# ultravideo/kvazaar

Hardware: AMD Instinct MI355X
Metric: CTUs/s (all-intra ultrafast hot path) (higher is better)
Workload: dtype u8/i16 (f64 RD costs); 1 GPU; 1920x1080 yuv420p 8-bit all-intra ultrafast CTU pass (kvz_hip_intra_frames), QP 22; ctus_per_frame=510, distinct_frames=8, wpp=True, parallelism=frames sharded over 1 GPU(s), no data-path collective

## Files before the change

### include/kvz_hip_dev.h

```cpp
#ifndef KVZ_HIP_DEV_H_
#define KVZ_HIP_DEV_H_

#include "kvz_hip_types.h"

#ifdef __cplusplus
extern "C" {
#endif

void *kvz_hip_dev_alloc(size_t bytes);
void  kvz_hip_dev_free(void *p);
void  kvz_hip_dev_upload(void *dev_dst, const void *host_src, size_t bytes);
void  kvz_hip_dev_download(void *host_dst, const void *dev_src, size_t bytes);
void  kvz_hip_dev_sync(void);
void  kvz_hip_dev_copy(void *dev_dst, const void *dev_src, size_t bytes);
void  kvz_hip_dev_timer_start(void);
float kvz_hip_dev_timer_stop(void);

int  kvz_hip_dev_sad_nxn(int n, const uint8_t *a, const uint8_t *b, int count, uint32_t *out);
int  kvz_hip_dev_satd_nxn(int n, const uint8_t *a, const uint8_t *b, int count, uint32_t *out);

int  kvz_hip_dev_transform(int kind, const int16_t *in, int16_t *tmp, int16_t *out, int count, int use_matrix_cores);

int  kvz_hip_dev_angular_pred(int log2_width, int mode, const uint8_t *ref_above, const uint8_t *ref_left, int count, uint8_t *out);

int  kvz_hip_dev_intra_select(int log2w, int nblk, const uint32_t *raw, const int8_t *preds, const double *mode_bits, int count, int32_t *winner);

int  kvz_hip_dev_cu8_units(int count, int from_coeffs, const int16_t *in, const int32_t *qp, int16_t *levels, int16_t *dequant, int16_t *resid);

int  kvz_hip_dev_satd8_blocks(const uint8_t *a, const uint8_t *b, int count, uint32_t *out);

void kvz_hip_dev_deblock_frames(uint8_t *frames, int width, int height, int n_frames, const uint8_t *cu_depth, int qp, int beta_offset_div2,
                                int tc_offset_div2);

typedef struct kvz_hip_cu_dbk {
  uint8_t type;
  uint8_t depth, tr_depth, part_size;
  uint8_t cbf_y;
  uint8_t mv_dir;
  int8_t  mv_ref[2];
  int16_t ref_id[2];
  int16_t mv[2][2];
} kvz_hip_cu_dbk;
void kvz_hip_dev_deblock_frames_inter(uint8_t *frames, int width, int height, int n_frames, const kvz_hip_cu_dbk *info, int qp, int beta_offset_div2,
                                      int tc_offset_div2, int slice_is_b);
// ... 131 lines not shown
```

### kvazaar_amd/csrc/kvz_ctu.hpp

```cpp
#pragma once
#include <type_traits>
#include "../../include/kvz_hip_types.h"
#include "kvz_ops.hpp"
#include "kvz_rdoq.hpp"
#include "kvz_recon.hpp"
#include "kvz_residual.hpp"
#include "kvz_select.hpp"

namespace kvz {

#define KVZ_CTU_THREADS 128
#ifdef KVZ_HOSTSIM
#define KVZ_FOR_THREADS(tid) for (int tid = 0; tid < KVZ_CTU_THREADS; ++tid)
#ifdef KVZ_HOSTSIM_COUNT_SYNCS
static unsigned long long g_kvz_syncs;
#define KVZ_SYNC() (++g_kvz_syncs)
#else
#define KVZ_SYNC()
#endif
#define KVZ_LDS_ADD(p, v) (*(p) += (v))
#else
#define KVZ_FOR_THREADS(tid) for (int tid = (threadIdx.x + lane_rot) & (KVZ_CTU_THREADS - 1), once_ = 1; once_; once_ = 0)
#define KVZ_SYNC() __syncthreads()
#define KVZ_LDS_ADD(p, v) atomicAdd((p), (v))
// ... 180 lines not shown
  u8 *cu_part = nullptr;
  u8 *cu_mode4 = nullptr;
  double *ctu_cost;
  unsigned long long *prof;
  u8 *border;
};
#define KVZ_BORDER_BYTES 512

template <bool CABAC> struct CtuSharedT {
  alignas(16) u8 org[1536];
  alignas(16) u8 dec[6144];
#if defined(KVZ_CTU_PROFILE) && !defined(KVZ_HOSTSIM)
  unsigned long long prof_rq[16];
  unsigned long long prof_acc[96];
  int prof_pu;
#endif
  CtuCu cu[4][64];
  u8 ref[3][2][68];
  u8 fref[2][68];
  union {
    struct {
      alignas(16) i16 tb_big[1536];
      alignas(16) u8 c1[1536];
    };
    struct {
      alignas(16) i16 tb_small[2 * 384];
      alignas(8) u8 org_t[256];
      alignas(16) u8 c2[384];
      alignas(16) i16 lv3_coeff[384];
      u8 mref[15][KVZ_MREF_STRIDE];
      u32 satd_raw[35][4];
    };
  };
  alignas(16) i16 lv2_coeff[384];
  alignas(16) i16 lv1_coeff[1536];
#ifdef KVZ_HOSTSIM
  alignas(16) i16 dct32[32 * 32];
#else
  alignas(16) i16 dct_small[64 + 16];
#endif
  u32 acc[16];
  int8_t preds[3];
  int best_mode;
  double cost[4], split_cost[4];
  double res[4];
  double child_bits[4];
// ... 5 lines not shown
  u8 dcval[3];
  int8_t mode_disp[35];
  int16_t mode_inv[35];
  QuantScalars qs[4][2];
  double mode_bits_cost[3];
  CtxSetT<CABAC> cab, pre[3], post2;
  float entropy_fbits[128];
  u8 ctx_lps[64];
};

using CtuShared = CtuSharedT<true>;
static_assert(__builtin_offsetof(CtuSharedT<true>, fref) == __builtin_offsetof(CtuSharedT<true>, ref) + 408 && __builtin_offsetof(CtuSharedT<false>, fref) == __builtin_offsetof(CtuSharedT<false>, ref) + 408,
              "Tables::mref_tab addresses the filtered references 408 bytes behind the unfiltered ones");
static_assert(KVZ_MREF_STRIDE == kMrefStride && KVZ_MREF_ORG == kMrefOrg && sizeof(((CtuSharedT<true> *)0)->ref[0][0]) == kMrefRefRow && kMrefFiltered == 408,
              "Tables::mref_tab (kvz_tables.hpp) is built for this layout of the reference arrays");
static_assert(KVZ_CTU_THREADS == 128, "two wavefronts per CTU: thread 64 is 'the other wavefront' (recon_cu8, eval_pu, wide_task, rdoq_unit, prices_coeffs, kHookThread), a 16x16 CU's "
                                      "128 (mode, block) pairs are one round of rough_search, plane_sums routes DPP rows per wavefront, and mref_pre[4] covers Tables::mref_tab's 510 entries");

KVZ_HD int plane_off(int c) { return c ? 3072 + (c << 10) : 0; }

struct RdoqLds {
  i32 ptab[2 * 148];
  u8 diag8[64];
  u8 mode4[4][64][4];
  u8 nb_mode4_left[16];
  u8 c4[96];
  alignas(8) i16 lv4_coeff[96];
  u8 pu_mode[4], pu_cbf[4];
  int pu_cbf_c[2];
  int a3x, a3y, n_pu;
// ... 565 lines not shown
        const int c = g < ny ? 0 : 1, i = g - (c == 0 ? 0 : ny);
        const int l2 = c ? log2w_c : log2w_y, n = 2 * (1 << l2) + 1, side = i >= n, k = side ? i - n : i;
        int qx, qy, dv;
        const bool have = ref_coords(l2, c, x, y, side, k, avail_top, avail_left, &qx, &qy);
        const lds_off off = rec_off(lv, c, qx, qy, &dv);
        s->ref[c][side][k] = have ? base[off] : (u8)128;
        if (c) s->ref[2][side][k] = have ? base[off + dv] : (u8)128;
      }
    }
    KVZ_SYNC();
    KVZ_FOR_THREADS(tid) {
      if (luma) {
        const int n = 2 * (1 << log2w_y) + 1;
        for (int i = tid; i < 2 * n; i += KVZ_CTU_THREADS) {
          const int side = i >= n, k = side ? i - n : i;
          const u8 *r = s->ref[0][side];
          u8 v;
          if (k == 0) v = (u8)((s->ref[0][1][1] + 2 * s->ref[0][1][0] + s->ref[0][0][1] + 2) / 4);
          else if (k == n - 1) v = r[k];
          else v = (u8)((r[k - 1] + 2 * r[k] + r[k + 1] + 2) / 4);
          s->fref[side][k] = v;
        }
      }
      const int c = mover_lane(tid) - (KVZ_CTU_THREADS - 3);
      if (c >= 0 && ((c == 0 && luma) || (c > 0 && chroma))) {
        const int l2 = c ? log2w_c : log2w_y, w = 1 << l2;
#ifdef KVZ_HOSTSIM
        s->dcval[c] = (u8)dc_value(l2, s->ref[c][0], s->ref[c][1]);
#else
        u32 sum = 0;
        for (int i = 0; i < w; i += 4) {
          u32 a, b;
          __builtin_memcpy(&a, &s->ref[c][0][1 + i], 4);
          __builtin_memcpy(&b, &s->ref[c][1][1 + i], 4);
          sum = __builtin_amdgcn_sad_u8(a, 0u, sum);
          sum = __builtin_amdgcn_sad_u8(b, 0u, sum);
// ... 44 lines not shown
      int d[8];
      for (int x = 0; x < 8; x++) d[x] = (int)pa[x] - (int)pb[x];
      int u0, u1, u2, u3;
      if (col & 4) { u0 = d[0] - d[4]; u1 = d[1] - d[5]; u2 = d[2] - d[6]; u3 = d[3] - d[7]; }
      else { u0 = d[0] + d[4]; u1 = d[1] + d[5]; u2 = d[2] + d[6]; u3 = d[3] + d[7]; }
      const int v0 = (col & 2) ? u0 - u2 : u0 + u2, v1 = (col & 2) ? u1 - u3 : u1 + u3;
      t[r] = (col & 1) ? v0 - v1 : v0 + v1;
    }
    KVZ_HAD8(t[0], t[1], t[2], t[3], t[4], t[5], t[6], t[7]);
    u32 sum = 0;
    for (int r = 0; r < 8; r++) sum += (u32)iabs(t[r]);
    return sum;
  }

#ifndef KVZ_HOSTSIM
  typedef unsigned short U16x2 __attribute__((ext_vector_type(2)));
  KVZ_DEV static U16x2 u16x2_of(unsigned v) { U16x2 r; __builtin_memcpy(&r, &v, 4); return r; }
  KVZ_DEV static U16x2 splat16(int v) { U16x2 r; r.x = (unsigned short)v; r.y = (unsigned short)v; return r; }
  KVZ_DEV static U16x2 widen(unsigned hi, unsigned lo, unsigned sel) { return u16x2_of(__builtin_amdgcn_perm(hi, lo, sel)); }
  KVZ_DEV static Pk16 as_pk16(U16x2 v) { Pk16 r; __builtin_memcpy(&r, &v, 4); return r; }
  KVZ_DEV static void widen8(const u8 *p, U16x2 out[4])
  {
    unsigned w[2];
    __builtin_memcpy(w, p, 8);
    out[0] = widen(0, w[0], 0x0c010c00u); out[1] = widen(0, w[0], 0x0c030c02u); out[2] = widen(0, w[1], 0x0c010c00u); out[3] = widen(0, w[1], 0x0c030c02u);
  }
#endif
  template <bool PAIR>
  KVZ_DEV u32 angular_block_satd(int log2w, int mode, int bx, int by, int xl, int yl, int half) const
  {
    const int w = 1 << log2w;
    const bool big = S32 && log2w == 5;
    const bool flat = mode < 2;
    const bool vertical = mode >= 18 || flat;
// ... 82 lines not shown
        sum += pk_absmax(pk_add(b0, b1)) + pk_absmax(pk_sub(b0, b1)) + pk_absmax(pk_add(b2, b3)) + pk_absmax(pk_sub(b2, b3));
        sum += pk_absmax(pk_add(b4, b5)) + pk_absmax(pk_sub(b4, b5)) + pk_absmax(pk_add(b6, b7)) + pk_absmax(pk_sub(b6, b7));
#else
        sum = pk_abs2_biased(pk_add(b0, b1), sum); sum = pk_abs2_biased(pk_sub(b0, b1), sum); sum = pk_abs2_biased(pk_add(b2, b3), sum); sum = pk_abs2_biased(pk_sub(b2, b3), sum);
        sum = pk_abs2_biased(pk_add(b4, b5), sum); sum = pk_abs2_biased(pk_sub(b4, b5), sum); sum = pk_abs2_biased(pk_add(b6, b7), sum); sum = pk_abs2_biased(pk_sub(b6, b7), sum);
#endif
      }
#ifndef KVZ_HOSTSIM
      return sum;
#endif
    }
    return 2 * sum;
  }

#ifndef KVZ_HOSTSIM
  KVZ_DEV u32 angular_group_satd(const SatdWalsh &wm, int log2w, int mode, int bx, int by, int xl, int yl, int half) const
  {
    const int w = 1 << log2w;
    const bool vertical = mode >= 18;
    const int disp = s->mode_disp[mode];
    const int p0 = vertical ? bx : by, q0 = vertical ? by : bx;
    const u8 *mr;
    if (disp < 0) mr = s->mref[mode - 11] + KVZ_MREF_ORG;
    else {
      const bool filt = imin(iabs(mode - 26), iabs(mode - 10)) > (log2w == 3 ? 7 : 1);
      mr = filt ? s->fref[vertical ? 0 : 1] : s->ref[0][vertical ? 0 : 1];
    }
    mr += p0 + 1;
    const u8 *org = vertical ? org_at(0, xl + bx, yl + by) : s->org_t + bx * w + by;
    const int ostride = vertical ? 32 : w;
    const u8 *side = vertical ? s->ref[0][1] : s->ref[0][0];
    const bool edge = disp == 0 && p0 == 0;
    const int r0 = 4 * half;
    unsigned rnd_bits = 0x10101010u;
    asm("" : "+v"(rnd_bits));
    dev_int4 p[2], o[2];
#pragma unroll
    for (int i = 0; i < 4; i++) {
      const int qa = q0 + r0 + i + 1, delta = qa * disp, di = delta >> 5, df = delta & 31;
      const u8 *m = mr + di;
      unsigned mw[2], ow[2];
      __builtin_memcpy(mw, m, 8);
      const unsigned m8 = m[8];
      __builtin_memcpy(ow, org + (r0 + i) * ostride, 8);
      const U16x2 c1 = splat16(df), c0 = splat16(32 - df), rnd = u16x2_of(rnd_bits);
      const U16x2 e0 = widen(0, mw[0], 0x0c020c00u), o0 = widen(0, mw[0], 0x0c030c01u), f0 = widen(mw[1], mw[0], 0x0c040c02u);
      const U16x2 e1 = widen(0, mw[1], 0x0c020c00u), o1 = widen(0, mw[1], 0x0c030c01u), f1 = widen(m8, mw[1], 0x0c040c02u);
      U16x2 v[4];
      v[0] = (e0 * c0 + (o0 * c1 + rnd)) >> (unsigned short)5; v[1] = (o0 * c0 + (f0 * c1 + rnd)) >> (unsigned short)5;
      v[2] = (e1 * c0 + (o1 * c1 + rnd)) >> (unsigned short)5; v[3] = (o1 * c0 + (f1 * c1 + rnd)) >> (unsigned short)5;
      if (edge) v[0].x = (unsigned short)iclip(128, 128 + 255, (int)v[0].x + (((int)side[qa] - (int)side[0]) >> 1));
      unsigned vw[4];
      __builtin_memcpy(vw, v, 16);
      p[i >> 1][2 * (i & 1)] = (int)__builtin_amdgcn_perm(vw[1], vw[0], 0x06020400u);
      p[i >> 1][2 * (i & 1) + 1] = (int)__builtin_amdgcn_perm(vw[3], vw[2], 0x06020400u);
      o[i >> 1][2 * (i & 1)] = (int)(ow[0] ^ 0x80808080u);
      o[i >> 1][2 * (i & 1) + 1] = (int)(ow[1] ^ 0x80808080u);
    }
    return satd8_group_mfma(wm, p, o);
  }

  KVZ_DEV u32 flat_block_satd8(int log2w, int mode, int bx, int by, int xl, int yl, int lane) const
  {
    const int w = 1 << log2w, r = lane & 7, y = by + r;
    U16x2 o[4], v[4];
    widen8(org_at(0, xl + bx, yl + y), o);
    if (mode == 0) {
      const u8 *top = s->fref[0], *left = s->fref[1];
      const int tr = top[w + 1], bl = left[w + 1], l = left[y + 1];
      U16x2 tp[4];
      widen8(top + bx + 1, tp);
      const U16x2 dl = splat16(tr - l), wy = splat16(w - 1 - y), hb = splat16((w - 1) * l + tr + (y + 1) * bl + w);
#pragma unroll
// ... 40 lines not shown
    u32 sum = pk_abs2_biased(d[3], pk_abs2_biased(d[2], pk_abs2_biased(d[1], pk_abs2_biased(d[0], 0))));
    sum += (u32)__builtin_amdgcn_update_dpp(0, (int)sum, 0xB1, 0xF, 0xF, true);
    sum += (u32)__builtin_amdgcn_update_dpp(0, (int)sum, 0x4E, 0xF, 0xF, true);
    sum += (u32)__builtin_amdgcn_update_dpp(0, (int)sum, 0x141, 0xF, 0xF, true);
    return sum;
  }
#endif

  template <int L2>
  KVZ_DEV void build_mref(int tid, const u32 *pre = nullptr)
  {
    constexpr int W = 1 << L2, NQ = 2 * W + 2, N = (15 * NQ + KVZ_CTU_THREADS - 1) / KVZ_CTU_THREADS;
    u8 vals[N];
    if constexpr (L2 != 5) {
      static_assert(N * KVZ_CTU_THREADS <= 512, "Tables::mref_tab rows");
      const u8 *src = &s->ref[0][0][0];
      u8 *dst = &s->mref[0][0];
      u32 e[N];
      for (int k = 0; k < N; k++) e[k] = pre ? pre[k] : tb->mref_tab[L2 - 3][tid + k * KVZ_CTU_THREADS];
      for (int k = 0; k < N; k++) vals[k] = src[e[k] & 0xffff];
      for (int k = 0; k < N; k++) dst[e[k] >> 16] = vals[k];
      return;
    }
    for (int k = 0; k < N; k++) {
      const int i = imin(tid + k * KVZ_CTU_THREADS, 15 * NQ - 1), mode = 11 + i / NQ, q = i % NQ - W;
      const bool vertical = mode >= 18, filt = luma_reads_filtered(L2, mode);
      const u8 *top = filt ? s->fref[0] : s->ref[0][0], *left = filt ? s->fref[1] : s->ref[0][1];
      const u8 *main_ref = vertical ? top : left, *side_ref = vertical ? left : top;
      const int idx = q >= 0 ? q : (128 + (-q) * (int)s->mode_inv[mode]) >> 8;
      vals[k] = (q >= 0 ? main_ref : side_ref)[imin(idx, 2 * W)];
    }
    for (int k = 0; k < N; k++) {
      const int i = tid + k * KVZ_CTU_THREADS;
      if (i < 15 * NQ) mref32()[(i / NQ) * KVZ_MREF32_STRIDE + KVZ_MREF32_ORG + i % NQ - W] = vals[k];
    }
  }
// ... 58 lines not shown
#undef KVZ_APPEND
#undef KVZ_RAW
    return final_mode;
#endif
  }
  template <class First>
  KVZ_DEV void rough_search(int lv, int x, int y, int depth, First first)
  {
    const int log2w = 6 - depth, w = 1 << log2w, xl = x - cx, yl = y - cy, nblk = (w >> 3) * (w >> 3);
#ifndef KVZ_HOSTSIM
    u32 mref_pre[4] = { 0, 0, 0, 0 };
    if (!(S32 && log2w == 5)) {
      const u32 *row = tb->mref_tab[log2w - 3] + ((threadIdx.x + lane_rot) & (KVZ_CTU_THREADS - 1));
      for (int k = 0; k < 4; k++) mref_pre[k] = row[k * KVZ_CTU_THREADS];
    }
#endif
    build_refs(lv, x, y, log2w, depth == 3 ? 2 : log2w - 1, true, true, first);
    if (S32 && log2w == 5) {
      KVZ_FOR_THREADS(tid) {
        if constexpr (S32) build_mref<5>(tid);
        u8 *ot = org_t32();
        for (int e = tid; e < 1024; e += KVZ_CTU_THREADS) ot[e] = *org_at(0, xl + (e >> 5), yl + (e & 31));
        for (int v = tid; v < 35; v += KVZ_CTU_THREADS) s->satd_raw[v][0] = 0;
        if (tid == KVZ_CTU_THREADS - 1) {
          int left, above;
          neighbour_pair(lv, x, y, &left, &above);
          mpm_candidates(y, left, above, s->preds);
        }
      }
      KVZ_SYNC();
// ... 11 lines not shown
          if (!(t & 1)) KVZ_LDS_ADD(&s->satd_raw[mode][0], (v + 2) >> 2);
        }
#endif
      }
    } else {
    KVZ_FOR_THREADS(tid) {
#ifdef KVZ_HOSTSIM
      if (log2w == 3) build_mref<3>(tid); else build_mref<4>(tid);
#else
      if (log2w == 3) build_mref<3>(tid, mref_pre); else build_mref<4>(tid, mref_pre);
#endif
      for (int e = tid; e < w * w; e += KVZ_CTU_THREADS) {
        const int ex = e >> log2w, ey = e & (w - 1);
        s->org_t[e] = *org_at(0, xl + ex, yl + ey);
      }
      if (tid == KVZ_CTU_THREADS - 1) {
        int left, above;
        neighbour_pair(lv, x, y, &left, &above);
        mpm_candidates(y, left, above, s->preds);
      }
    }
    KVZ_SYNC();
    KVZ_PROF(KVZ_P_PRED35);
    KVZ_FOR_THREADS(tid) {
      const int lb = 2 * (log2w - 3);
#ifdef KVZ_HOSTSIM
      for (int t = tid; t < 35 * nblk; t += KVZ_CTU_THREADS) {
        const int mi = t >> lb, mode = mi < 33 ? mi + 2 : mi - 33, b = t & (nblk - 1), bx = (b & ((w >> 3) - 1)) * 8, by = (b >> (log2w - 3)) * 8;
        s->satd_raw[mode][b] = angular_block_satd<false>(log2w, mode, bx, by, xl, yl, 0);
      }
#else
      if (log2w == 4 || tid < 64) {
        const int lane = tid & 63;
        const SatdWalsh wm = satd8_walsh(tb, lane);
        for (int g = log2w == 4 ? 2 * (tid >> 6) : 0, ge = g + (log2w == 4 ? 2 : 1); g < ge; g++) {
          const int p = 32 * g + (lane & 31), mode = 2 + (p >> lb), b = p & (nblk - 1), bx = (b & ((w >> 3) - 1)) * 8, by = (b >> (log2w - 3)) * 8;
          const u32 v = angular_group_satd(wm, log2w, mode, bx, by, xl, yl, lane >> 5);
          if (lane < 32) s->satd_raw[mode][b] = v;
        }
      }
      {
        const int t = KVZ_CTU_THREADS - 1 - tid;
        if (t < 24 * nblk) {
          const int mb = t >> 3, mi = mb >> lb, mode = mi == 0 ? 34 : mi - 1, b = mb & (nblk - 1), bx = (b & ((w >> 3) - 1)) * 8, by = (b >> (log2w - 3)) * 8;
          const u32 v = flat_block_satd8(log2w, mode, bx, by, xl, yl, tid);
          if ((tid & 7) == 0) s->satd_raw[mode][b] = v;
        }
      }
#endif
    }
    }
    KVZ_SYNC();
    KVZ_PROF(KVZ_P_SATD);
// ... 1847 lines not shown
```

### kvazaar_amd/csrc/kvz_dev.hpp

```cpp
#pragma once
#include <hip/hip_runtime.h>

#include <functional>
#include <mutex>
#include <chrono>
#include <vector>

#include "../../include/kvz_hip_dev.h"
#include "kvz_mfma.hpp"
#include "kvz_ops.hpp"
#include "kvz_sao.hpp"
#include "kvz_entropy.hpp"
#include "kvz_select.hpp"
#include "kvz_recon.hpp"
#include "kvz_tables.hpp"

namespace kvz {

__device__ __forceinline__ u32 load_u32_any(const u8 *p) { u32 v; __builtin_memcpy(&v, p, 4); return v; }
template <int G> __device__ __forceinline__ u32 group_sum(u32 v)
{
  for (int off = G / 2; off > 0; off >>= 1) v += __shfl_down(v, off, G);
  return v;
}
// ... 273 lines not shown
  const int c = tid < 64 ? 0 : (tid < 80 ? 1 : 2), e = tid < 64 ? tid : (tid & 15), q = live ? qp[unit] : 0;
  Cu8MatRow fwd = {}, inv = {};
  if (tid < 64) cu8_matrix_rows<3>(tb, e, fwd, inv); else cu8_matrix_rows<2>(tb, e, fwd, inv);
  for (int stage = 1; stage <= 5; stage++) {
    if (live) {
      if (tid < 64) dev_cu8_lane<3>(stage, c, e, t[half], from_coeffs, q, fwd, inv, in + o, levels + o, dequant + o, resid + o);
      else dev_cu8_lane<2>(stage, c, e, t[half], from_coeffs, q, fwd, inv, in + o, levels + o, dequant + o, resid + o);
    }
    __syncthreads();
  }
}

__global__ void __launch_bounds__(256) dev_satd8_blocks_kernel(const Tables *tb, const u8 *a, const u8 *b, const int count, u32 *out)
{
  dev_satd8_blocks_wave(tb, a, b, count, out, (int)(blockIdx.x * 4 + (threadIdx.x >> 6)), (int)(threadIdx.x & 63));
}

template <int L2> __global__ void __launch_bounds__(256) dev_angular_kernel(const u8 *above, const u8 *left, const int count, const int mode, u8 *out)
{
  constexpr int W = 1 << L2, NG = kAngularGroupsPerLane, GPB = W * W / 4, BLOCKS = 256 * NG / GPB, RS = 2 * W + 1, ES = (2 * W + 1 + 8 + 3) & ~3;
  constexpr int RAW = (BLOCKS * RS + 3 + 3) / 4 + 2;
  __shared__ u32 s_raw[2][RAW];
  __shared__ alignas(8) u8 s_ext[BLOCKS][ES];
  __shared__ u32 s_tile[BLOCKS * W * W / 4];
  const int disp_tab[9] = { 0, 2, 5, 9, 13, 17, 21, 26, 32 };
  const int inv_tab[9] = { 0, 4096, 1638, 910, 630, 482, 390, 315, 256 };
  const bool vertical = mode >= 18;
  const int mode_disp = vertical ? mode - 26 : 10 - mode, ad = iabs(mode_disp);
  const int disp = mode_disp < 0 ? -disp_tab[ad] : disp_tab[ad], inv = inv_tab[ad];
  const long blk0 = (long)blockIdx.x * BLOCKS;
// ... 865 lines not shown
}

int kvz_hip_dev_intra_select(int log2w, int nblk, const uint32_t *raw, const int8_t *preds, const double *mode_bits, int count, int32_t *winner)
{
  if (!((log2w == 3 && nblk == 1) || (log2w == 4 && nblk == 4))) { fprintf(stderr, "kvz_hip_dev_intra_select: unsupported log2w=%d nblk=%d\n", log2w, nblk); return -1; }
  if (count <= 0) return 0;
  KVZ_DEV_LAUNCH(kvz::dev_intra_select_kernel, ((long)count + 3) / 4 * 256, raw, preds, mode_bits, count, log2w, nblk, winner);
  return 0;
}

int kvz_hip_dev_cu8_units(int count, int from_coeffs, const int16_t *in, const int32_t *qp, int16_t *levels, int16_t *dequant, int16_t *resid)
{
  if (count < 0 || (from_coeffs != 0 && from_coeffs != 1)) { fprintf(stderr, "kvz_hip_dev_cu8_units: count=%d from_coeffs=%d\n", count, from_coeffs); return -1; }
  if (count == 0) return 0;
  KVZ_DEV_LAUNCH(kvz::dev_cu8_units_kernel, ((long)count + 1) / 2 * 256, in, qp, count, from_coeffs, kvz::device_tables(), levels, dequant, resid);
  return 0;
}

int kvz_hip_dev_satd8_blocks(const uint8_t *a, const uint8_t *b, int count, uint32_t *out)
{
  if (count < 0) { fprintf(stderr, "kvz_hip_dev_satd8_blocks: count=%d\n", count); return -1; }
  KVZ_DEV_LAUNCH(kvz::dev_satd8_blocks_kernel, ((long)count + 31) / 32 * 64, kvz::device_tables(), a, b, count, out);
  return 0;
}

void kvz_hip_dev_deblock_frames(uint8_t *frames, int width, int height, int n_frames, const uint8_t *cu_depth, int qp, int beta_offset_div2,
                                int tc_offset_div2)
{
  kvz::deblock_frames_on(be().stream, frames, width, height, n_frames, cu_depth, qp, beta_offset_div2, tc_offset_div2);
}
// ... 1035 lines not shown
```

### kvazaar_amd/csrc/kvz_mfma.hpp

```cpp
#pragma once
#include <hip/hip_runtime.h>

#include "kvz_ops.hpp"

namespace kvz {

typedef int dev_int4 __attribute__((ext_vector_type(4)));
typedef int dev_int16 __attribute__((ext_vector_type(16)));

__device__ __forceinline__ void dev_byte_planes(int v0, int v1, int v2, int v3, u32 &lo, u32 &hi)
{
  const u32 t01 = __builtin_amdgcn_perm((u32)v1, (u32)v0, 0x05010400u), t23 = __builtin_amdgcn_perm((u32)v3, (u32)v2, 0x05010400u);
  lo = __builtin_amdgcn_perm(t23, t01, 0x05040100u) ^ 0x80808080u;
  hi = __builtin_amdgcn_perm(t23, t01, 0x07060302u);
}

template <int N> struct DevMma;
template <> struct DevMma<16> {
  static constexpr int NREG = 4;
  static __device__ __forceinline__ int idx(int lane) { return lane & 15; }
  static __device__ __forceinline__ int row(int lane, int r) { return 4 * (lane >> 4) + r; }
  static __device__ __forceinline__ int k0(int lane, int) { return 4 * (lane >> 4); }
  static constexpr int STEPS = 1;
};
// ... 140 lines not shown
  for (int tile = 0; tile < 2; tile++) {
    dev_int16 t;
#pragma unroll
    for (int r = 0; r < 16; r++) t[r] = kSatdBias;
    t = __builtin_amdgcn_mfma_i32_32x32x32_i8(tile ? w.neg : w.pos, p[1], t, 0, 0, 0);
    t = __builtin_amdgcn_mfma_i32_32x32x32_i8(w.pos, p[0], t, 0, 0, 0);
    t = __builtin_amdgcn_mfma_i32_32x32x32_i8(tile ? w.pos : w.neg, o[1], t, 0, 0, 0);
    t = __builtin_amdgcn_mfma_i32_32x32x32_i8(w.neg, o[0], t, 0, 0, 0);
#pragma unroll
    for (int r = 0; r < 16; r++) sums[r & 1] = __builtin_amdgcn_sad_u16((u32)t[r], (u32)kSatdBias, sums[r & 1]);
  }
  const u32 sum = sums[0] + sums[1];
  const auto both = __builtin_amdgcn_permlane32_swap(sum, sum, false, false);
  return both[0] + both[1];
}
__device__ __forceinline__ void dev_satd8_blocks_wave(const Tables *tb, const u8 *a, const u8 *bsrc, int count, u32 *out, int group, int lane)
{
  const long blk = 32l * group + (lane & 31);
  const bool live = blk < count;
  dev_int4 p[2] = {}, o[2] = {};
  if (live) {
    const dev_int4 *pa = reinterpret_cast<const dev_int4 *>(a + 64 * blk + 32 * (lane >> 5)), *po = reinterpret_cast<const dev_int4 *>(bsrc + 64 * blk + 32 * (lane >> 5));
    p[0] = pa[0]; p[1] = pa[1]; o[0] = po[0]; o[1] = po[1];
  }
#pragma unroll
  for (int q = 0; q < 2; q++) { p[q] ^= (int)0x80808080u; o[q] ^= (int)0x80808080u; }
  const u32 v = satd8_group_mfma(satd8_walsh(tb, lane), p, o);
  if (live && lane < 32) out[blk] = v;
}

// ... 2 lines not shown
```

### kvazaar_amd/csrc/kvz_ops.hpp

```cpp
#pragma once
#include <stdint.h>

#ifdef KVZ_HOSTSIM
#define KVZ_DEV inline
#define KVZ_ATOMIC_ADD(p, v) (*(p) += (v))
#else
#include <hip/hip_runtime.h>
#define KVZ_DEV __device__ __forceinline__
#define KVZ_ATOMIC_ADD(p, v) atomicAdd((p), (v))
#endif

namespace kvz {

typedef uint8_t u8;
typedef int16_t i16;
typedef uint16_t u16;
typedef uint32_t u32;
typedef int32_t i32;

#ifdef KVZ_HOSTSIM
#define KVZ_HD inline
#else
#define KVZ_HD __host__ __device__ __forceinline__
#endif
// ... 13 lines not shown
  return __builtin_amdgcn_sdot2(va, vb, c, false);
}
#endif
#ifndef KVZ_HOSTSIM
KVZ_DEV int row16_sum(int v)
{
  v += __builtin_amdgcn_update_dpp(0, v, 0x118, 0xF, 0xF, true);
  v += __builtin_amdgcn_update_dpp(0, v, 0x114, 0xF, 0xF, true);
  v += __builtin_amdgcn_update_dpp(0, v, 0x112, 0xF, 0xF, true);
  v += __builtin_amdgcn_update_dpp(0, v, 0x111, 0xF, 0xF, true);
  return v;
}
#endif

constexpr unsigned kMrefStride = 36, kMrefOrg = 16, kMrefRefRow = 68, kMrefFiltered = 408;

struct Tables {
  i16 dct[4][32 * 32];
  i16 dst4[16];
  alignas(16) int8_t dct_i8[2][2][32 * 32];
  alignas(16) i32 dct_sum[2][2][32];
  alignas(16) int8_t bd_i8[3][2][16 * 16];
  alignas(16) i32 bd_sum[3][2][16];
  u32 small_pairs[3][2][8][4];
  u32 pairs16[2][16][8];
  u32 scan[3][4][1024];
  u8 avail_top[16][16], avail_left[16][16];
  u8 ctx_next[2][128];
  u32 mref_tab[2][512];
  u8 diag8[64];
  u32 entropy_bits[128];
  int8_t luma_filter[4][8];
  int8_t chroma_filter[8][4];
  alignas(16) u32 satd_walsh[64][8];
};

KVZ_HD u32 satd_walsh_word(int lane, int q)
{
  const int i = lane & 31, h = lane >> 5;
  const u32 base = 0x01010101u ^ ((i & 1) ? 0xfe00fe00u : 0u) ^ ((i & 2) ? 0xfefe0000u : 0u);
  const int minus = (((i >> 4) & h) ^ ((i >> 3) & (q >> 1)) ^ ((i >> 2) & q)) & 1;
  return base ^ (minus ? 0xfefefefeu : 0u);
}


struct SadRectOp {
  const u8 *a; int a_stride; long a_bstride;
  const u8 *b; int b_stride; long b_bstride;
  int w, h;
  int clamp, ref_w, ref_h, ref_x, ref_y;
// ... 583 lines not shown
```

### kvazaar_amd/csrc/kvz_tables.hpp

```cpp
#pragma once
#include <string.h>

#include "kvz_recon.hpp"
#include "kvz_syntax.hpp"

namespace kvz {

inline int dct32_entry(int k, int n)
{
  static const int mag[32] = { 64, 90, 90, 90, 89, 88, 87, 85, 83, 82, 80, 78, 75, 73, 70, 67,
                               64, 61, 57, 54, 50, 46, 43, 38, 36, 31, 25, 22, 18, 13, 9,  4 };
  if (k == 0) return 64;
  const int m = (k * (2 * n + 1)) % 128;
  if (m < 32) return mag[m];
  if (m < 64) return -mag[64 - m];
  if (m < 96) return -mag[m - 64];
  return mag[128 - m];
}

inline void scan_pattern(int type, int size, int *xs, int *ys)
{
  int n = 0;
  if (type == 0) {
    for (int d = 0; d < 2 * size - 1; d++)
// ... 85 lines not shown
  }
  for (int l2 = 3; l2 <= 4; l2++) {
    static const int inv_tab[9] = { 0, 4096, 1638, 910, 630, 482, 390, 315, 256 };
    const int w = 1 << l2, nq = 2 * w + 2;
    for (int i = 0; i < 15 * nq; i++) {
      const int mode = 11 + i / nq, q = i % nq - w, vertical = mode >= 18, md = vertical ? mode - 26 : 10 - mode, ad = md < 0 ? -md : md;
      const bool filt = luma_reads_filtered(l2, mode);
      int idx = q >= 0 ? q : (128 + (-q) * inv_tab[ad]) >> 8;
      if (idx > 2 * w) idx = 2 * w;
      const int main_side = vertical ? 0 : 1, side = q >= 0 ? main_side : 1 - main_side;
      const unsigned src = (filt ? kMrefFiltered : 0u) + kMrefRefRow * side + idx, dst = kMrefStride * (i / nq) + kMrefOrg + i % nq - w;
      t->mref_tab[l2 - 3][i] = src | dst << 16;
    }
    for (int i = 15 * nq; i < 512; i++) t->mref_tab[l2 - 3][i] = t->mref_tab[l2 - 3][15 * nq - 1];
  }
  for (int lane = 0; lane < 64; lane++)
    for (int q = 0; q < 4; q++) { t->satd_walsh[lane][q] = satd_walsh_word(lane, q); t->satd_walsh[lane][4 + q] = satd_walsh_word(lane, q) ^ 0xfefefefeu; }
  static const i16 dst4[16] = { 29, 55, 74, 84, 74, 74, 0, -74, 84, -29, -74, 55, 55, -84, 74, -29 };
  memcpy(t->dst4, dst4, sizeof dst4);
  for (int kind = 0; kind < 3; kind++) {
    const int n = kind == 1 ? 8 : 4;
    const i16 *m = kind == 2 ? t->dst4 : t->dct[kind == 1 ? 1 : 0];
    for (int g = 0; g < 16 / n; g++)
      for (int k = 0; k < n; k++)
        for (int j = 0; j < n; j++) {
          t->bd_i8[kind][0][(g * n + k) * 16 + g * n + j] = (int8_t)m[k * n + j];
          t->bd_i8[kind][1][(g * n + j) * 16 + g * n + k] = (int8_t)m[k * n + j];
          t->bd_sum[kind][0][g * n + k] += m[k * n + j];
          t->bd_sum[kind][1][g * n + j] += m[k * n + j];
        }
// ... 103 lines not shown
```

### kvazaar_amd/dev.py

```python
import ctypes as C

import numpy as np

TRANSFORM_KINDS = {"dct4": 0, "dct8": 1, "dct16": 2, "dct32": 3, "dst4": 4, "idct4": 5, "idct8": 6, "idct16": 7, "idct32": 8, "idst4": 9}
TRANSFORM_SIZE = {0: 4, 1: 8, 2: 16, 3: 32, 4: 4, 5: 4, 6: 8, 7: 16, 8: 32, 9: 4}


class Dev:
    def __init__(self, cdll):
        self.lib = l = cdll
        vp, sz, ci = C.c_void_p, C.c_size_t, C.c_int
        l.kvz_hip_dev_alloc.restype = vp; l.kvz_hip_dev_alloc.argtypes = [sz]
        l.kvz_hip_dev_free.restype = None; l.kvz_hip_dev_free.argtypes = [vp]
        l.kvz_hip_dev_upload.restype = None; l.kvz_hip_dev_upload.argtypes = [vp, vp, sz]
        l.kvz_hip_dev_download.restype = None; l.kvz_hip_dev_download.argtypes = [vp, vp, sz]
        l.kvz_hip_dev_sync.restype = None; l.kvz_hip_dev_sync.argtypes = []
        l.kvz_hip_dev_timer_start.restype = None; l.kvz_hip_dev_timer_start.argtypes = []
        l.kvz_hip_dev_timer_stop.restype = C.c_float; l.kvz_hip_dev_timer_stop.argtypes = []
        for f in (l.kvz_hip_dev_sad_nxn, l.kvz_hip_dev_satd_nxn):
            f.restype = None; f.argtypes = [ci, vp, vp, ci, vp]
        l.kvz_hip_dev_transform.restype = None; l.kvz_hip_dev_transform.argtypes = [ci, vp, vp, vp, ci, ci]
        l.kvz_hip_dev_angular_pred.restype = None; l.kvz_hip_dev_angular_pred.argtypes = [ci, ci, vp, vp, ci, vp]
        l.kvz_hip_dev_intra_select.restype = ci; l.kvz_hip_dev_intra_select.argtypes = [ci, ci, vp, vp, vp, ci, vp]
        l.kvz_hip_dev_cu8_units.restype = ci; l.kvz_hip_dev_cu8_units.argtypes = [ci, ci, vp, vp, vp, vp, vp]
        l.kvz_hip_dev_satd8_blocks.restype = ci; l.kvz_hip_dev_satd8_blocks.argtypes = [vp, vp, ci, vp]

    def put(self, a):
        a = np.ascontiguousarray(a)
        p = self.lib.kvz_hip_dev_alloc(a.nbytes)
        self.lib.kvz_hip_dev_upload(p, a.ctypes.data, a.nbytes)
        return p

    def copy_in(self, p, a):
        a = np.ascontiguousarray(a)
        self.lib.kvz_hip_dev_upload(p, a.ctypes.data, a.nbytes)

    def empty(self, nbytes):
        return self.lib.kvz_hip_dev_alloc(nbytes)

    def get(self, p, shape, dtype):
# ... 8 lines not shown
```

Measured before the change: 3.364 million CTUs/s.

## Precompute per-lane angular SATD row descriptors in a table for rough search

Replaces the per-lane angular prediction address and weight arithmetic in the rough intra SATD search with a precomputed table (satd_rows) of window offsets, edge-byte offsets, source offsets and fractional weights, loaded once per CU. Edge filtering of DC-displacement modes becomes a precomputed XOR byte in LDS, and the interpolation switches to 8-bit fixed-point weights with a byte-permute instead of a shift. Source rows for SATD are loaded once and shared across both mode groups on 16x16 CUs. It also adds a standalone rough_rows test kernel and moves helper functions into shared headers, at the cost of a larger constant table and extra LDS bytes inside an existing union.

```diff
diff --git a/include/kvz_hip_dev.h b/include/kvz_hip_dev.h
--- a/include/kvz_hip_dev.h
+++ b/include/kvz_hip_dev.h
@@ -28,6 +28,8 @@
 int  kvz_hip_dev_cu8_units(int count, int from_coeffs, const int16_t *in, const int32_t *qp, int16_t *levels, int16_t *dequant, int16_t *resid);
 
 int  kvz_hip_dev_satd8_blocks(const uint8_t *a, const uint8_t *b, int count, uint32_t *out);
+
+int  kvz_hip_dev_rough_rows(int log2w, const uint8_t *top, const uint8_t *left, int count, uint8_t *out);
 
 void kvz_hip_dev_deblock_frames(uint8_t *frames, int width, int height, int n_frames, const uint8_t *cu_depth, int qp, int beta_offset_div2,
                                 int tc_offset_div2);
diff --git a/kvazaar_amd/csrc/kvz_ctu.hpp b/kvazaar_amd/csrc/kvz_ctu.hpp
--- a/kvazaar_amd/csrc/kvz_ctu.hpp
+++ b/kvazaar_amd/csrc/kvz_ctu.hpp
@@ -218,6 +218,7 @@
   unsigned long long prof_rq[16];
   unsigned long long prof_acc[96];
   int prof_pu;
+  int prof_pad_[3];
 #endif
   CtuCu cu[4][64];
   u8 ref[3][2][68];
@@ -234,6 +235,7 @@
       alignas(16) i16 lv3_coeff[384];
       u8 mref[15][KVZ_MREF_STRIDE];
       u32 satd_raw[35][4];
+      u8 edge_x[36];
     };
   };
   alignas(16) i16 lv2_coeff[384];
@@ -269,6 +271,15 @@
               "Tables::mref_tab addresses the filtered references 408 bytes behind the unfiltered ones");
 static_assert(KVZ_MREF_STRIDE == kMrefStride && KVZ_MREF_ORG == kMrefOrg && sizeof(((CtuSharedT<true> *)0)->ref[0][0]) == kMrefRefRow && kMrefFiltered == 408,
               "Tables::mref_tab (kvz_tables.hpp) is built for this layout of the reference arrays");
+#define KVZ_FROM_REF(T, member) (__builtin_offsetof(T, member) - __builtin_offsetof(T, ref))
+static_assert(KVZ_FROM_REF(CtuSharedT<true>, mref) == kMrefExtended && KVZ_FROM_REF(CtuSharedT<false>, mref) == kMrefExtended && KVZ_FROM_REF(CtuSharedT<true>, org_t) == kSatdSrcT &&
+              KVZ_FROM_REF(CtuSharedT<false>, org_t) == kSatdSrcT && KVZ_FROM_REF(CtuSharedT<true>, edge_x) == kSatdEdge && KVZ_FROM_REF(CtuSharedT<false>, edge_x) == kSatdEdge,
+              "Tables::satd_rows (kvz_tables.hpp) addresses the extended references, the transposed source block and the edge bytes from CtuShared::ref");
+static_assert(sizeof(((CtuSharedT<true> *)0)->edge_x) >= 1 + 2 * 16 && __builtin_offsetof(CtuSharedT<true>, edge_x) + sizeof(((CtuSharedT<true> *)0)->edge_x) <= __builtin_offsetof(CtuSharedT<true>, lv2_coeff) &&
+              __builtin_offsetof(CtuSharedT<true>, org) == 0 && __builtin_offsetof(CtuSharedT<true>, ref) % 8 == 0 && __builtin_offsetof(CtuSharedT<true>, org_t) % 8 == 0,
+              "the edge bytes of a 16x16 CU fit, behind satd_raw and inside the union; source rows (offsets that are multiples of 8 from org / org_t) are 8-byte aligned");
+static_assert(__builtin_offsetof(CtuSharedT<true>, lv2_coeff) - __builtin_offsetof(CtuSharedT<true>, tb_big) == 3072 + 1536, "the union is as large as its 32x32 regime: edge_x added nothing");
+#undef KVZ_FROM_REF
 static_assert(KVZ_CTU_THREADS == 128, "two wavefronts per CTU: thread 64 is 'the other wavefront' (recon_cu8, eval_pu, wide_task, rdoq_unit, prices_coeffs, kHookThread), a 16x16 CU's "
                                       "128 (mode, block) pairs are one round of rough_search, plane_sums routes DPP rows per wavefront, and mref_pre[4] covers Tables::mref_tab's 510 entries");
 
@@ -864,12 +875,7 @@
         const int n = 2 * (1 << log2w_y) + 1;
         for (int i = tid; i < 2 * n; i += KVZ_CTU_THREADS) {
           const int side = i >= n, k = side ? i - n : i;
-          const u8 *r = s->ref[0][side];
-          u8 v;
-          if (k == 0) v = (u8)((s->ref[0][1][1] + 2 * s->ref[0][1][0] + s->ref[0][0][1] + 2) / 4);
-          else if (k == n - 1) v = r[k];
-          else v = (u8)((r[k - 1] + 2 * r[k] + r[k + 1] + 2) / 4);
-          s->fref[side][k] = v;
+          s->fref[side][k] = luma_filtered_ref(&s->ref[0][0][0], n, i);
         }
       }
       const int c = mover_lane(tid) - (KVZ_CTU_THREADS - 3);
@@ -944,10 +950,6 @@
   }
 
 #ifndef KVZ_HOSTSIM
-  typedef unsigned short U16x2 __attribute__((ext_vector_type(2)));
-  KVZ_DEV static U16x2 u16x2_of(unsigned v) { U16x2 r; __builtin_memcpy(&r, &v, 4); return r; }
-  KVZ_DEV static U16x2 splat16(int v) { U16x2 r; r.x = (unsigned short)v; r.y = (unsigned short)v; return r; }
-  KVZ_DEV static U16x2 widen(unsigned hi, unsigned lo, unsigned sel) { return u16x2_of(__builtin_amdgcn_perm(hi, lo, sel)); }
   KVZ_DEV static Pk16 as_pk16(U16x2 v) { Pk16 r; __builtin_memcpy(&r, &v, 4); return r; }
   KVZ_DEV static void widen8(const u8 *p, U16x2 out[4])
   {
@@ -1060,49 +1062,10 @@
   }
 
 #ifndef KVZ_HOSTSIM
-  KVZ_DEV u32 angular_group_satd(const SatdWalsh &wm, int log2w, int mode, int bx, int by, int xl, int yl, int half) const
-  {
-    const int w = 1 << log2w;
-    const bool vertical = mode >= 18;
-    const int disp = s->mode_disp[mode];
-    const int p0 = vertical ? bx : by, q0 = vertical ? by : bx;
-    const u8 *mr;
-    if (disp < 0) mr = s->mref[mode - 11] + KVZ_MREF_ORG;
-    else {
-      const bool filt = imin(iabs(mode - 26), iabs(mode - 10)) > (log2w == 3 ? 7 : 1);
-      mr = filt ? s->fref[vertical ? 0 : 1] : s->ref[0][vertical ? 0 : 1];
-    }
-    mr += p0 + 1;
-    const u8 *org = vertical ? org_at(0, xl + bx, yl + by) : s->org_t + bx * w + by;
-    const int ostride = vertical ? 32 : w;
-    const u8 *side = vertical ? s->ref[0][1] : s->ref[0][0];
-    const bool edge = disp == 0 && p0 == 0;
-    const int r0 = 4 * half;
-    unsigned rnd_bits = 0x10101010u;
-    asm("" : "+v"(rnd_bits));
-    dev_int4 p[2], o[2];
-#pragma unroll
-    for (int i = 0; i < 4; i++) {
-      const int qa = q0 + r0 + i + 1, delta = qa * disp, di = delta >> 5, df = delta & 31;
-      const u8 *m = mr + di;
-      unsigned mw[2], ow[2];
-      __builtin_memcpy(mw, m, 8);
-      const unsigned m8 = m[8];
-      __builtin_memcpy(ow, org + (r0 + i) * ostride, 8);
-      const U16x2 c1 = splat16(df), c0 = splat16(32 - df), rnd = u16x2_of(rnd_bits);
-      const U16x2 e0 = widen(0, mw[0], 0x0c020c00u), o0 = widen(0, mw[0], 0x0c030c01u), f0 = widen(mw[1], mw[0], 0x0c040c02u);
-      const U16x2 e1 = widen(0, mw[1], 0x0c020c00u), o1 = widen(0, mw[1], 0x0c030c01u), f1 = widen(m8, mw[1], 0x0c040c02u);
-      U16x2 v[4];
-      v[0] = (e0 * c0 + (o0 * c1 + rnd)) >> (unsigned short)5; v[1] = (o0 * c0 + (f0 * c1 + rnd)) >> (unsigned short)5;
-      v[2] = (e1 * c0 + (o1 * c1 + rnd)) >> (unsigned short)5; v[3] = (o1 * c0 + (f1 * c1 + rnd)) >> (unsigned short)5;
-      if (edge) v[0].x = (unsigned short)iclip(128, 128 + 255, (int)v[0].x + (((int)side[qa] - (int)side[0]) >> 1));
-      unsigned vw[4];
-      __builtin_memcpy(vw, v, 16);
-      p[i >> 1][2 * (i & 1)] = (int)__builtin_amdgcn_perm(vw[1], vw[0], 0x06020400u);
-      p[i >> 1][2 * (i & 1) + 1] = (int)__builtin_amdgcn_perm(vw[3], vw[2], 0x06020400u);
-      o[i >> 1][2 * (i & 1)] = (int)(ow[0] ^ 0x80808080u);
-      o[i >> 1][2 * (i & 1) + 1] = (int)(ow[1] ^ 0x80808080u);
-    }
+  KVZ_DEV u32 angular_group_satd(const SatdWalsh &wm, const dev_int4 rows[2], const dev_int4 o[2]) const
+  {
+    dev_int4 p[2];
+    satd_rows_predict(&s->ref[0][0][0], rows, p);
     return satd8_group_mfma(wm, p, o);
   }
 
@@ -1173,12 +1136,9 @@
     u8 vals[N];
     if constexpr (L2 != 5) {
       static_assert(N * KVZ_CTU_THREADS <= 512, "Tables::mref_tab rows");
-      const u8 *src = &s->ref[0][0][0];
-      u8 *dst = &s->mref[0][0];
       u32 e[N];
       for (int k = 0; k < N; k++) e[k] = pre ? pre[k] : tb->mref_tab[L2 - 3][tid + k * KVZ_CTU_THREADS];
-      for (int k = 0; k < N; k++) vals[k] = src[e[k] & 0xffff];
-      for (int k = 0; k < N; k++) dst[e[k] >> 16] = vals[k];
+      mref_copy<N>(&s->ref[0][0][0], e);
       return;
     }
     for (int k = 0; k < N; k++) {
@@ -1267,6 +1227,15 @@
       const u32 *row = tb->mref_tab[log2w - 3] + ((threadIdx.x + lane_rot) & (KVZ_CTU_THREADS - 1));
       for (int k = 0; k < 4; k++) mref_pre[k] = row[k * KVZ_CTU_THREADS];
     }
+    dev_int4 rows_pre[2][2] = {};
+    {
+      const int t = (threadIdx.x + lane_rot) & (KVZ_CTU_THREADS - 1);
+      if (log2w == 4 || (log2w == 3 && t < 64)) {
+        const dev_int4 *row = reinterpret_cast<const dev_int4 *>(tb->satd_rows[log2w == 4 ? 1 + 2 * (t >> 6) : 0][t & 63]);
+        rows_pre[0][0] = row[0]; rows_pre[0][1] = row[1];
+        if (log2w == 4) { rows_pre[1][0] = row[2 * 64]; rows_pre[1][1] = row[2 * 64 + 1]; }
+      }
+    }
 #endif
     build_refs(lv, x, y, log2w, depth == 3 ? 2 : log2w - 1, true, true, first);
     if (S32 && log2w == 5) {
@@ -1308,6 +1277,12 @@
         const int ex = e >> log2w, ey = e & (w - 1);
         s->org_t[e] = *org_at(0, xl + ex, yl + ey);
       }
+#ifndef KVZ_HOSTSIM
+      if (tid <= 2 * w) {
+        const u8 xv = satd_edge_byte(&s->ref[0][0][0], log2w, tid & (2 * w - 1));
+        s->edge_x[tid == 2 * w ? 0 : 1 + tid] = tid == 2 * w ? (u8)0 : xv;
+      }
+#endif
       if (tid == KVZ_CTU_THREADS - 1) {
         int left, above;
         neighbour_pair(lv, x, y, &left, &above);
@@ -1327,10 +1302,14 @@
       if (log2w == 4 || tid < 64) {
         const int lane = tid & 63;
         const SatdWalsh wm = satd8_walsh(tb, lane);
-        for (int g = log2w == 4 ? 2 * (tid >> 6) : 0, ge = g + (log2w == 4 ? 2 : 1); g < ge; g++) {
-          const int p = 32 * g + (lane & 31), mode = 2 + (p >> lb), b = p & (nblk - 1), bx = (b & ((w >> 3) - 1)) * 8, by = (b >> (log2w - 3)) * 8;
-          const u32 v = angular_group_satd(wm, log2w, mode, bx, by, xl, yl, lane >> 5);
-          if (lane < 32) s->satd_raw[mode][b] = v;
+        dev_int4 o[2];
+        satd_rows_source(&s->ref[0][0][0], org_at(0, xl, yl), rows_pre[0], o);
+        const int p = (log2w == 4 ? 64 * (tid >> 6) : 0) + (lane & 31), mode = 2 + (p >> lb), b = p & (nblk - 1);
+        const u32 v0 = angular_group_satd(wm, rows_pre[0], o);
+        if (lane < 32) s->satd_raw[mode][b] = v0;
+        if (log2w == 4) {
+          const u32 v1 = angular_group_satd(wm, rows_pre[1], o);
+          if (lane < 32) s->satd_raw[mode + 8][b] = v1;
         }
       }
       {
diff --git a/kvazaar_amd/csrc/kvz_dev.hpp b/kvazaar_amd/csrc/kvz_dev.hpp
--- a/kvazaar_amd/csrc/kvz_dev.hpp
+++ b/kvazaar_amd/csrc/kvz_dev.hpp
@@ -311,6 +311,50 @@
 __global__ void __launch_bounds__(256) dev_satd8_blocks_kernel(const Tables *tb, const u8 *a, const u8 *b, const int count, u32 *out)
 {
   dev_satd8_blocks_wave(tb, a, b, count, out, (int)(blockIdx.x * 4 + (threadIdx.x >> 6)), (int)(threadIdx.x & 63));
+}
+
+template <int L2> __global__ void __launch_bounds__(256) dev_rough_rows_kernel(const Tables *tb, const u8 *top, const u8 *left, const int count, u8 *out)
+{
+  constexpr int W = 1 << L2, N = 2 * W + 1, NM = (15 * (2 * W + 2) + 127) / 128, LB = 2 * (L2 - 3), NBLK = 1 << LB;
+  static_assert(2 * N <= 128 && NM * 128 <= 512, "a lane per reference sample; Tables::mref_tab rows");
+  __shared__ alignas(16) u8 lds[2][(kSatdEdge + 1 + 2 * 16 + 15) & ~15u];
+  const int half = threadIdx.x >> 7, tid = threadIdx.x & 127, lane = tid & 63;
+  const long cu = 2l * blockIdx.x + half;
+  const bool live = cu < count;
+  u8 *ref0 = lds[half];
+  const int side = tid >= N, k = side ? tid - N : tid;
+  if (live && tid < 2 * N) ref0[kMrefRefRow * side + k] = (side ? left : top)[cu * N + k];
+  __syncthreads();
+  if (live && tid < 2 * N) ref0[kMrefFiltered + kMrefRefRow * side + k] = luma_filtered_ref(ref0, N, tid);
+  __syncthreads();
+  if (live) {
+    u32 e[NM];
+    for (int j = 0; j < NM; j++) e[j] = tb->mref_tab[L2 - 3][tid + j * 128];
+    mref_copy<NM>(ref0, e);
+    if (tid <= 2 * W) {
+      const u8 xv = satd_edge_byte(ref0, L2, tid & (2 * W - 1));
+      ref0[kSatdEdge + (tid == 2 * W ? 0 : 1 + tid)] = tid == 2 * W ? (u8)0 : xv;
+    }
+  }
+  __syncthreads();
+  if (!live || (L2 == 3 && tid >= 64)) return;
+#pragma unroll
+  for (int j = 0; j < (L2 == 4 ? 2 : 1); j++) {
+    const int g = L2 == 4 ? 2 * (tid >> 6) + j : 0, pr = 32 * g + (lane & 31), mode = 2 + (pr >> LB), b = pr & (NBLK - 1);
+    const dev_int4 *row = reinterpret_cast<const dev_int4 *>(tb->satd_rows[L2 == 4 ? 1 + g : 0][lane]);
+    const dev_int4 e[2] = { row[0], row[1] };
+    dev_int4 p[2];
+    satd_rows_predict(ref0, e, p);
+    u8 *o = out + ((cu * 32 + (mode - 2)) * NBLK + b) * 64;
+#pragma unroll
+    for (int i = 0; i < 4; i++)
+#pragma unroll
+      for (int x = 0; x < 8; x++) {
+        const int r = 4 * (lane >> 5) + i;
+        const u8 v = (u8)(((u32)p[i >> 1][2 * (i & 1) + (x >> 2)] >> (8 * (x & 3))) ^ 0x80);
+        o[mode >= 18 ? 8 * r + x : 8 * x + r] = v;
+      }
+  }
 }
 
 template <int L2> __global__ void __launch_bounds__(256) dev_angular_kernel(const u8 *above, const u8 *left, const int count, const int mode, u8 *out)
@@ -1206,6 +1250,14 @@
   if (count < 0 || (from_coeffs != 0 && from_coeffs != 1)) { fprintf(stderr, "kvz_hip_dev_cu8_units: count=%d from_coeffs=%d\n", count, from_coeffs); return -1; }
   if (count == 0) return 0;
   KVZ_DEV_LAUNCH(kvz::dev_cu8_units_kernel, ((long)count + 1) / 2 * 256, in, qp, count, from_coeffs, kvz::device_tables(), levels, dequant, resid);
+  return 0;
+}
+
+int kvz_hip_dev_rough_rows(int log2w, const uint8_t *top, const uint8_t *left, int count, uint8_t *out)
+{
+  if (count < 0 || (log2w != 3 && log2w != 4)) { fprintf(stderr, "kvz_hip_dev_rough_rows: log2w=%d count=%d\n", log2w, count); return -1; }
+  if (log2w == 3) KVZ_DEV_LAUNCH(kvz::dev_rough_rows_kernel<3>, ((long)count + 1) / 2 * 256, kvz::device_tables(), top, left, count, out);
+  else KVZ_DEV_LAUNCH(kvz::dev_rough_rows_kernel<4>, ((long)count + 1) / 2 * 256, kvz::device_tables(), top, left, count, out);
   return 0;
 }
 
diff --git a/kvazaar_amd/csrc/kvz_mfma.hpp b/kvazaar_amd/csrc/kvz_mfma.hpp
--- a/kvazaar_amd/csrc/kvz_mfma.hpp
+++ b/kvazaar_amd/csrc/kvz_mfma.hpp
@@ -178,6 +178,47 @@
   const auto both = __builtin_amdgcn_permlane32_swap(sum, sum, false, false);
   return both[0] + both[1];
 }
+typedef unsigned short U16x2 __attribute__((ext_vector_type(2)));
+__device__ __forceinline__ U16x2 u16x2_of(unsigned v) { U16x2 r; __builtin_memcpy(&r, &v, 4); return r; }
+__device__ __forceinline__ U16x2 splat16(int v) { U16x2 r; r.x = (unsigned short)v; r.y = (unsigned short)v; return r; }
+__device__ __forceinline__ U16x2 widen(unsigned hi, unsigned lo, unsigned sel) { return u16x2_of(__builtin_amdgcn_perm(hi, lo, sel)); }
+
+__device__ __forceinline__ void satd_rows_predict(const u8 *ref0, const dev_int4 e[2], dev_int4 p[2])
+{
+  unsigned rnd_bits = 0x80808080u;
+  asm("" : "+v"(rnd_bits));
+#pragma unroll
+  for (int i = 0; i < 4; i++) {
+    const unsigned w0 = (unsigned)e[i >> 1][2 * (i & 1)], w1 = (unsigned)e[i >> 1][2 * (i & 1) + 1];
+    unsigned mw[3];
+    static_assert(kSatdWindow == sizeof mw, "the window read");
+    __builtin_memcpy(mw, ref0 + (w0 & 0xffff), sizeof mw);
+    const unsigned ex = ref0[w0 >> 16];
+    const U16x2 wt = u16x2_of(w1), c1 = wt.xx, c0 = splat16(256) - c1, rnd = u16x2_of(rnd_bits);
+    const U16x2 e0 = widen(0, mw[0], 0x0c020c00u), o0 = widen(0, mw[0], 0x0c030c01u), f0 = widen(mw[1], mw[0], 0x0c040c02u);
+    const U16x2 e1 = widen(0, mw[1], 0x0c020c00u), o1 = widen(0, mw[1], 0x0c030c01u), f1 = widen(mw[2], mw[1], 0x0c040c02u);
+    U16x2 v[4];
+    v[0] = e0 * c0 + (o0 * c1 + rnd); v[1] = o0 * c0 + (f0 * c1 + rnd);
+    v[2] = e1 * c0 + (o1 * c1 + rnd); v[3] = o1 * c0 + (f1 * c1 + rnd);
+    unsigned vw[4];
+    __builtin_memcpy(vw, v, 16);
+    p[i >> 1][2 * (i & 1)] = (int)(__builtin_amdgcn_perm(vw[1], vw[0], 0x07030501u) ^ ex);
+    p[i >> 1][2 * (i & 1) + 1] = (int)__builtin_amdgcn_perm(vw[3], vw[2], 0x07030501u);
+  }
+}
+__device__ __forceinline__ void satd_rows_source(const u8 *ref0, const u8 *cu_org, const dev_int4 e[2], dev_int4 o[2])
+{
+  const u8 *base = ((unsigned)e[0][1] >> 16 & kSatdSrcVertical) ? cu_org : ref0;
+#pragma unroll
+  for (int i = 0; i < 4; i++) {
+    const unsigned src = (unsigned)e[i >> 1][2 * (i & 1) + 1] >> 16 & (kSatdSrcVertical - 1);
+    unsigned ow[2];
+    __builtin_memcpy(ow, __builtin_assume_aligned(base + src, 8), 8);
+    o[i >> 1][2 * (i & 1)] = (int)(ow[0] ^ 0x80808080u);
+    o[i >> 1][2 * (i & 1) + 1] = (int)(ow[1] ^ 0x80808080u);
+  }
+}
+
 __device__ __forceinline__ void dev_satd8_blocks_wave(const Tables *tb, const u8 *a, const u8 *bsrc, int count, u32 *out, int group, int lane)
 {
   const long blk = 32l * group + (lane & 31);
diff --git a/kvazaar_amd/csrc/kvz_ops.hpp b/kvazaar_amd/csrc/kvz_ops.hpp
--- a/kvazaar_amd/csrc/kvz_ops.hpp
+++ b/kvazaar_amd/csrc/kvz_ops.hpp
@@ -51,6 +51,7 @@
 #endif
 
 constexpr unsigned kMrefStride = 36, kMrefOrg = 16, kMrefRefRow = 68, kMrefFiltered = 408;
+constexpr unsigned kMrefExtended = 3488, kSatdSrcT = 2080, kSatdEdge = 4588, kSatdWindow = 12, kSatdSrcVertical = 0x8000;
 
 struct Tables {
   i16 dct[4][32 * 32];
@@ -70,7 +71,44 @@
   int8_t luma_filter[4][8];
   int8_t chroma_filter[8][4];
   alignas(16) u32 satd_walsh[64][8];
-};
+  alignas(16) u32 satd_rows[5][64][8];
+};
+
+struct SatdRow { unsigned window, edge, src; int df; bool vertical; };
+KVZ_HD SatdRow satd_row_of(u32 w0, u32 w1)
+{
+  SatdRow r;
+  r.window = w0 & 0xffff; r.edge = w0 >> 16; r.df = (int)(w1 & 0xffff) >> 3; r.vertical = (w1 >> 16 & kSatdSrcVertical) != 0; r.src = w1 >> 16 & (kSatdSrcVertical - 1);
+  return r;
+}
+KVZ_HD void satd_row_walk(const u8 *ref0, u32 w0, u32 w1, u8 out[8])
+{
+  const SatdRow r = satd_row_of(w0, w1);
+  const u8 *m = ref0 + r.window;
+  for (int k = 0; k < 8; k++) out[k] = (u8)(((32 - r.df) * m[k] + r.df * m[k + 1] + 16) >> 5);
+  out[0] ^= ref0[r.edge];
+}
+KVZ_HD u8 satd_edge_byte(const u8 *ref0, int log2w, int i)
+{
+  const int o = i >> log2w, q = i & ((1 << log2w) - 1);
+  const u8 *side = ref0 + kMrefRefRow * (1 - o);
+  const int main1 = ref0[kMrefRefRow * o + 1];
+  return (u8)(iclip(0, 255, main1 + (((int)side[q + 1] - (int)side[0]) >> 1)) ^ main1);
+}
+template <int N> KVZ_DEV void mref_copy(u8 *ref0, const u32 e[N])
+{
+  u8 vals[N];
+  for (int k = 0; k < N; k++) vals[k] = ref0[e[k] & 0xffff];
+  for (int k = 0; k < N; k++) ref0[kMrefExtended + (e[k] >> 16)] = vals[k];
+}
+KVZ_HD u8 luma_filtered_ref(const u8 *ref0, int n, int i)
+{
+  const int side = i >= n, k = side ? i - n : i;
+  const u8 *r = ref0 + kMrefRefRow * side;
+  if (k == 0) return (u8)((ref0[kMrefRefRow + 1] + 2 * ref0[kMrefRefRow] + ref0[1] + 2) / 4);
+  if (k == n - 1) return r[k];
+  return (u8)((r[k - 1] + 2 * r[k] + r[k + 1] + 2) / 4);
+}
 
 KVZ_HD u32 satd_walsh_word(int lane, int q)
 {
diff --git a/kvazaar_amd/csrc/kvz_tables.hpp b/kvazaar_amd/csrc/kvz_tables.hpp
--- a/kvazaar_amd/csrc/kvz_tables.hpp
+++ b/kvazaar_amd/csrc/kvz_tables.hpp
@@ -1,4 +1,5 @@
 #pragma once
+#include <assert.h>
 #include <string.h>
 
 #include "kvz_recon.hpp"
@@ -123,6 +124,24 @@
     }
     for (int i = 15 * nq; i < 512; i++) t->mref_tab[l2 - 3][i] = t->mref_tab[l2 - 3][15 * nq - 1];
   }
+  for (int l2 = 3; l2 <= 4; l2++)
+    for (int g = 0; g < (l2 == 3 ? 1 : 4); g++)
+      for (int lane = 0; lane < 64; lane++)
+        for (int i = 0; i < 4; i++) {
+          static const int disp_tab[9] = { 0, 2, 5, 9, 13, 17, 21, 26, 32 };
+          const int w = 1 << l2, lb = 2 * (l2 - 3), p = 32 * g + (lane & 31), mode = 2 + (p >> lb), b = p & ((1 << lb) - 1);
+          const int bx = (b & ((w >> 3) - 1)) * 8, by = (b >> (l2 - 3)) * 8, r = 4 * (lane >> 5) + i;
+          const int vertical = mode >= 18, md = vertical ? mode - 26 : 10 - mode, disp = md < 0 ? -disp_tab[-md] : disp_tab[md];
+          const int p0 = vertical ? bx : by, q0 = vertical ? by : bx, qa = q0 + r + 1, delta = qa * disp, df = delta & 31, di = (delta - df) / 32;
+          const unsigned row = disp < 0 ? kMrefExtended + kMrefStride * (mode - 11) : (luma_reads_filtered(l2, mode) ? kMrefFiltered : 0u) + kMrefRefRow * (vertical ? 0 : 1);
+          const int at = (disp < 0 ? (int)kMrefOrg : 0) + p0 + 1 + di;
+          assert(at >= 0 && at + (int)kSatdWindow <= (int)(disp < 0 ? kMrefStride : kMrefRefRow));
+          const unsigned edge = disp == 0 && p0 == 0 ? kSatdEdge + 1 + (vertical ? 0 : w) + qa - 1 : kSatdEdge;
+          const unsigned src = vertical ? kSatdSrcVertical | (unsigned)((by + r) * 32 + bx) : kSatdSrcT + (unsigned)((bx + r) * w + by);
+          u32 *e = t->satd_rows[l2 == 3 ? 0 : 1 + g][lane] + 2 * i;
+          e[0] = (row + (unsigned)at) | edge << 16;
+          e[1] = (unsigned)(8 * df) | src << 16;
+        }
   for (int lane = 0; lane < 64; lane++)
     for (int q = 0; q < 4; q++) { t->satd_walsh[lane][q] = satd_walsh_word(lane, q); t->satd_walsh[lane][4 + q] = satd_walsh_word(lane, q) ^ 0xfefefefeu; }
   static const i16 dst4[16] = { 29, 55, 74, 84, 74, 74, 0, -74, 84, -29, -74, 55, 55, -84, 74, -29 };
diff --git a/kvazaar_amd/dev.py b/kvazaar_amd/dev.py
--- a/kvazaar_amd/dev.py
+++ b/kvazaar_amd/dev.py
@@ -24,6 +24,8 @@
         l.kvz_hip_dev_intra_select.restype = ci; l.kvz_hip_dev_intra_select.argtypes = [ci, ci, vp, vp, vp, ci, vp]
         l.kvz_hip_dev_cu8_units.restype = ci; l.kvz_hip_dev_cu8_units.argtypes = [ci, ci, vp, vp, vp, vp, vp]
         l.kvz_hip_dev_satd8_blocks.restype = ci; l.kvz_hip_dev_satd8_blocks.argtypes = [vp, vp, ci, vp]
+        if hasattr(l, "kvz_hip_dev_rough_rows"):
+            l.kvz_hip_dev_rough_rows.restype = ci; l.kvz_hip_dev_rough_rows.argtypes = [ci, vp, vp, ci, vp]
 
     def put(self, a):
         a = np.ascontiguousarray(a)
```

Measured after the change: 3.578 million CTUs/s (median of 6 runs). 1.06x the previous value.
